# erdc/petsc-dev

Measured on AMD Instinct MI355X. Metric: KSP CG+Jacobi iterations/s x unknowns (3-D 7-pt Poisson, 256^3 rows per GPU); ksp_its_per_sec and spmv_gbps are BASELINE.json's two quantities, higher is better.
Workload: dtype f64

## Files before the change

### petsc-dev_amd/csrc/spmv_csr.hip

```cpp
#include "common.hpp"
#include <map>
#include <array>
#include <memory>
#include <vector>
#include <stdlib.h>
#include <string.h>

#ifndef SPMV_THREADS
#define SPMV_THREADS 256
#endif
#ifndef SPMV_NT
#define SPMV_NT 1
#endif
#ifndef SPMV_REMAP
#define SPMV_REMAP 2
#endif
#ifndef SPMV_CH
#define SPMV_CH 32
#endif
#ifndef SPMV_MINWAVES
#define SPMV_MINWAVES 1
#endif
#ifndef SPMV_SEQ_AVG
#define SPMV_SEQ_AVG 16
#endif
#define SPMV_GJ_CAP 960
#define SPMV_BLOCK_NNZ (8 * SPMV_THREADS)
#define SPMV_BLOCK_CAP (SPMV_BLOCK_NNZ - 2)
#define SPMV_BLOCK_ROWS SPMV_THREADS
#define SPMV_PAIRS (SPMV_BLOCK_NNZ / (2 * SPMV_THREADS))
#define SPMV_WAVES (SPMV_THREADS / MI355X_WAVE)
#if SPMV_NT
#define SPMV_LOAD(p) __builtin_nontemporal_load(p)
#else
#define SPMV_LOAD(p) (*(p))
#endif
static_assert(SPMV_THREADS == 256 && MI355X_WAVE == 64, "one lane per row of a block with byte row markers, 256-entry offset table and 512-entry pattern tables staged one / two per lane");
static_assert(SPMV_REMAP == 0 || SPMV_REMAP == 2, "SPMV_REMAP == 1 (each XCD walks a contiguous eighth of the row blocks) was removed: only the plain kernel ever had it; use 0 or 2");

typedef double v2d __attribute__((ext_vector_type(2)));
typedef int v2i __attribute__((ext_vector_type(2)));

struct mi355x_spmv_plan_s {
  int nrows;
  int nblocks;
  int nlong;
  int2 *d_rowblk;
  int *d_rows;
  unsigned char *d_idx8;
  int *d_offtab;
  int ntab;
  unsigned int *d_prow;
  int *d_pattab;
  int npat, use_pat;
  unsigned int *d_pruns;
  int nruncoded, use_runs;
  int ch;
  unsigned short *d_vrow;
  int *d_vpattab;
  double *d_vpatval;
  int nvpat, vtablen, vpat_valid, use_vpat;
  double *d_dotpart;
  int ndotpart;
  int pairsum;
  int4 *d_rowblk4;
  int *d_goff;
  int *d_gj;
  int ngroups;
  long ngj;
};


static inline int rowblock_grid(int nblocks, int ch) {
  const int per = SPMV_REMAP == 2 ? MI355X_NXCD * ch : 1;
  return ((nblocks + per - 1) / per) * per;
}
__device__ __forceinline__ int rowblock_of_workgroup(int ch) {
  if (SPMV_REMAP != 2) return blockIdx.x;
  const int xcd = blockIdx.x % MI355X_NXCD, slot = blockIdx.x / MI355X_NXCD;
  return ((slot / ch) * MI355X_NXCD + xcd) * ch + (slot % ch);
}

struct row_lanes { int tpr, r, sub; };
__device__ __forceinline__ row_lanes lanes_per_row(int nrows, int nnz, int tid, bool short_rows_one_lane = true) {
  int lg = 0;
  while (lg < 6 && ((nrows * 2) << lg) <= SPMV_THREADS) ++lg;
  if (short_rows_one_lane && nnz <= SPMV_SEQ_AVG * nrows) lg = 0;
  return {1 << lg, tid >> lg, tid & ((1 << lg) - 1)};
}

__device__ __forceinline__ int pair_k(int k0, int tid, int p) { return (k0 & ~1) + 2 * tid + p * 2 * SPMV_THREADS; }
template <typename PAIR, typename T> __device__ __forceinline__ PAIR load_pair(const T *a, int k0, int k1, int k) {
  return SPMV_LOAD(reinterpret_cast<const PAIR *>(a + (k < k1 ? k : (k0 & ~1))));
}
struct pair_src { int kk, s0, s1; };
__device__ __forceinline__ pair_src pair_source(int k, int k0, int k1) {
  const bool in = k < k1;
  const bool v0 = in && k >= k0, v1 = in && (k + 1 < k1);
  return {in ? k : (k0 & ~1), v0 ? 0 : (in ? 1 : (k0 & 1)), v1 ? 1 : (in ? 0 : (k0 & 1))};
}
__device__ __forceinline__ void park_pair(double *stage, int k, int k0, int k1, double a, double b) {
  stage[(k >= k0 && k < k1) ? k - k0 : SPMV_BLOCK_NNZ - 1] = a;
  stage[(k + 1 < k1) ? k + 1 - k0 : SPMV_BLOCK_NNZ - 1] = b;
}

template <class PROD> __device__ __forceinline__ double accumulate8(double sum, int k, int end, int pairsum, PROD prod) {
  if (!pairsum) {
#pragma unroll
    for (int j = 0; j < 8; ++j) { const double u = sum + prod(j); sum = (k + j < end) ? u : sum; }
  } else {
#pragma unroll
    for (int j = 0; j < 8; j += 2) {
      const double pa = prod(j), pb = prod(j + 1);
      const double inc = (k + j + 1 < end) ? pa + pb : pa;
      const double u = sum + inc;
      sum = (k + j < end) ? u : sum;
    }
  }
  return sum;
}
__device__ __forceinline__ double row_sum_lds(const double *prod, int rs, int re, double sum, int pairsum) {
  auto run = [&](int pairs) {
    for (int k = rs; k < re; k += 8) {
      double t[8];
#pragma unroll
      for (int j = 0; j < 8; ++j) t[j] = prod[(k + j < re) ? k + j : re - 1];
      sum = accumulate8(sum, k, re, pairs, [&](int j) { return t[j]; });
    }
  };
  if (!pairsum) run(0); else run(1);
  return sum;
}

template <int ADD> __device__ __forceinline__ double spmv_out(double yv, double t, double dv = 1.0) { return ADD == 3 ? dv * (yv + t) : (ADD == 1 ? yv + t : (ADD == 2 ? yv * t : t)); }
template <int ADD> __device__ __forceinline__ double spmv_empty(double yv, double dv = 1.0) { return ADD == 3 ? dv * yv : (ADD == 1 ? yv : (ADD == 2 ? yv * 0.0 : 0.0)); }
template <int ADD> __device__ __forceinline__ double spmv_fin(double yv, double s, double dv = 1.0) { return ADD == 3 ? dv * s : (ADD == 2 ? yv * s : s); }
static inline int spmv_y_streams(long nrows) { return (size_t)nrows * sizeof(double) >= ((size_t)256 << 20); }
__device__ __forceinline__ void spmv_store(double *p, double v, bool nt) { if (nt) __builtin_nontemporal_store(v, p); else *p = v; }

template <int ADD>
__device__ __forceinline__ double row_result_lds(const double *prod, int tpr, int sub, bool has_row, int rs, int re, double yv, double dv,
                                                 int pairsum, double *dst, bool nt) {
  double res = 0.0;
  if (tpr == 1) {
    if (has_row) { res = spmv_fin<ADD>(yv, row_sum_lds(prod, rs, re, (ADD & 1) ? yv : 0.0, pairsum), dv); spmv_store(dst, res, nt); }
  } else {
    double sum = 0.0;
    if (has_row) for (int k = rs + sub; k < re; k += tpr) sum += prod[k];
    for (int off = tpr >> 1; off > 0; off >>= 1) sum += __shfl_down(sum, off, MI355X_WAVE);
    if (has_row && sub == 0) { res = re == rs ? spmv_empty<ADD>(yv, dv) : spmv_out<ADD>(yv, sum, dv); spmv_store(dst, res, nt); }
  }
  return res;
}

template <int NW> __device__ __forceinline__ double workgroup_sum_ordered(double v) {
  __shared__ double wave_slot[NW];
  const int tid = threadIdx.x;
  v = wave_sum(v);
  if ((tid & (MI355X_WAVE - 1)) == 0) wave_slot[tid / MI355X_WAVE] = v;
  __syncthreads();
  double t = 0.0;
  if (tid == 0) {
    t = wave_slot[0];
// ... 64 lines not shown
    for (int p = 0; p < SPMV_PAIRS; ++p) {
      const pair_src s = pair_source(pair_k(k0, tid, p), k0, k1);
      xa[p] = x[s.s0 ? c[p].y : c[p].x];
      xb[p] = x[s.s1 ? c[p].y : c[p].x];
    }
#pragma unroll
    for (int p = 0; p < SPMV_PAIRS; ++p) park_pair(prod, pair_k(k0, tid, p), k0, k1, v[p].x * xa[p], v[p].y * xb[p]);
  } else {
    for (int k = k0 + tid; k < k1; k += SPMV_THREADS)
      prod[k - k0] = SPMV_LOAD(aa + k) * x[SPMV_LOAD(aj + k)];
  }
  __syncthreads();

  const int rs = r < nrows ? a0 - k0 : 0, re = r < nrows ? a1 - k0 : 0;
  row_result_lds<ADD>(prod, tpr, sub, r < nrows, rs, re, ysum, dv, pairsum, yout + orow, nt);
}

template <int ADD, bool DOT>
__global__ __launch_bounds__(SPMV_THREADS, SPMV_MINWAVES) void spmv_csr_rowblock_idx8_kernel(
    const int2 *__restrict__ rowblk, int nblocks, const int *__restrict__ ai, const unsigned char *__restrict__ idx8,
    const int *__restrict__ offtab_g, int ntab, const double *__restrict__ aa, const double *__restrict__ x,
    const double *yin, double *yout, double *__restrict__ dotpart, int pairsum) {
  __shared__ double prod[SPMV_BLOCK_NNZ];
  __shared__ unsigned char rowof[SPMV_BLOCK_NNZ];
  __shared__ int offtab[256];
  static_assert(!(DOT && ADD != 0), "the x'y by-product is provided for y = A x only");
  const int lb = rowblock_of_workgroup(SPMV_CH);
  if (lb >= nblocks) return;
  const int2 b0 = rowblk[lb];
  const int2 b1 = rowblk[lb + 1];
  const int r0 = b0.x, r1 = b1.x, k0 = b0.y, k1 = b1.y;
  const int nnz = k1 - k0;
  const int nrows = r1 - r0;
  const int tid = threadIdx.x;
  const int tabv = offtab_g[tid];
  (void)ntab;
  if (nnz == 0) {
    if (tid < nrows) yout[r0 + tid] = spmv_empty<ADD>(ADD ? yin[r0 + tid] : 0.0);
    if (DOT && tid == 0) dotpart[lb] = 0.0;
    return;
  }

  const row_lanes rl = lanes_per_row(nrows, nnz, tid);
  const int tpr = rl.tpr, r = rl.r, sub = rl.sub;
  const int rc = r < nrows ? r : nrows - 1;
  const int a0 = ai[r0 + rc], a1 = ai[r0 + rc + 1];
  double ysum = 0.0;
  if (ADD) ysum = yin[r0 + rc];
  double xrow = 0.0;
  if (DOT) xrow = x[r0 + rc];
  v2d v[SPMV_PAIRS];
  unsigned int ix[SPMV_PAIRS];
#pragma unroll
  for (int p = 0; p < SPMV_PAIRS; ++p) {
    v[p] = load_pair<v2d>(aa, k0, k1, pair_k(k0, tid, p));
    ix[p] = load_pair<unsigned short>(idx8, k0, k1, pair_k(k0, tid, p));
  }
  const int rs = r < nrows ? a0 - k0 : 0, re = r < nrows ? a1 - k0 : 0;
  for (int k = rs + sub; k < re; k += tpr) rowof[k] = (unsigned char)r;
  offtab[tid] = tabv;
  __syncthreads();
  double xa[SPMV_PAIRS], xb[SPMV_PAIRS];
#pragma unroll
  for (int p = 0; p < SPMV_PAIRS; ++p) {
    const pair_src s = pair_source(pair_k(k0, tid, p), k0, k1);
    xa[p] = x[r0 + rowof[s.kk + s.s0 - k0] + offtab[(ix[p] >> (8 * s.s0)) & 0xff]];
    xb[p] = x[r0 + rowof[s.kk + s.s1 - k0] + offtab[(ix[p] >> (8 * s.s1)) & 0xff]];
  }
#pragma unroll
  for (int p = 0; p < SPMV_PAIRS; ++p) park_pair(prod, pair_k(k0, tid, p), k0, k1, v[p].x * xa[p], v[p].y * xb[p]);
  __syncthreads();
  const double yval = row_result_lds<ADD>(prod, tpr, sub, r < nrows, rs, re, ysum, 1.0, pairsum, yout + r0 + rc, false);
  if (DOT) {
    const double t = workgroup_sum_ordered<SPMV_WAVES>((r < nrows && sub == 0) ? yval * xrow : 0.0);
    if (tid == 0) dotpart[lb] = t;
  }
}

#define SPMV_PAT_CAP 512
#define SPMV_RUNS 4
#define SPMV_RUN_WORDS (2 * SPMV_RUNS)
#define SPMV_RUN_NONE 0xffffu
static_assert(SPMV_RUNS == 4, "the kernel loads a block's runs as two uint4");
template <int ADD, bool DOT>
__global__ __launch_bounds__(SPMV_THREADS, SPMV_MINWAVES) void spmv_csr_rowblock_pat_kernel(
    const int2 *__restrict__ rowblk, int nblocks, const unsigned int *__restrict__ prow, const uint4 *__restrict__ pruns,
    const int *__restrict__ pattab_g, const double *__restrict__ aa, const double *__restrict__ x, const double *yin, double *yout,
    double *__restrict__ dotpart, int pairsum, int ch, int nty) {
  __shared__ double vs[SPMV_BLOCK_NNZ];
  __shared__ int pattab[SPMV_PAT_CAP];
  const int lb = rowblock_of_workgroup(ch);
  if (lb >= nblocks) return;
  const int2 b0 = rowblk[lb];
  const int2 b1 = rowblk[lb + 1];
  uint4 d0 = make_uint4(0u, SPMV_RUN_NONE, 0u, SPMV_RUN_NONE), d1 = d0;
  if (pruns) { d0 = pruns[2 * (size_t)lb]; d1 = pruns[2 * (size_t)lb + 1]; }
  const int r0 = b0.x, r1 = b1.x, k0 = b0.y, k1 = b1.y;
  const int nrows = r1 - r0;
  const int tid = threadIdx.x;
  const int t0 = pattab_g[tid], t1 = pattab_g[tid + SPMV_THREADS];
  if (k1 == k0) {
    if (tid < nrows) yout[r0 + tid] = spmv_empty<ADD>(ADD ? yin[r0 + tid] : 0.0);
    if (DOT && tid == 0) dotpart[lb] = 0.0;
    return;
  }
  const int rc = tid < nrows ? tid : nrows - 1;
  const bool coded = (d0.y & 0xffffu) == 0u;
  unsigned int pw = d0.x, rn = d0.y;
  if ((unsigned int)rc >= (d0.w & 0xffffu)) { pw = d0.z; rn = d0.w; }
  if ((unsigned int)rc >= (d1.y & 0xffffu)) { pw = d1.x; rn = d1.y; }
  if ((unsigned int)rc >= (d1.w & 0xffffu)) { pw = d1.z; rn = d1.w; }
  if (!coded) pw = prow[r0 + rc];
  const int pst = (int)(pw & 0xffffu);
  const int rs = (int)(pw >> 16) + (rc - (int)(rn & 0xffffu)) * (int)(rn >> 16);
  double ysum = 0.0;
  if (ADD) ysum = yin[r0 + rc];
  v2d v[SPMV_PAIRS];
#pragma unroll
  for (int p = 0; p < SPMV_PAIRS; ++p) v[p] = load_pair<v2d>(aa, k0, k1, pair_k(k0, tid, p));
  pattab[tid] = t0;
  pattab[tid + SPMV_THREADS] = t1;
#pragma unroll
  for (int p = 0; p < SPMV_PAIRS; ++p) park_pair(vs, pair_k(k0, tid, p), k0, k1, v[p].x, v[p].y);
  __syncthreads();
  if (!DOT && tid >= nrows) return;
  const int len = tid < nrows ? (coded ? (int)(rn >> 16) : pattab[pst]) : 0;
  const long xbase = (long)r0 + rc;
  double sum = (ADD == 1) ? ysum : 0.0;
  for (int q0 = 0; q0 < len; q0 += 8) {
    double xv[8], av[8];
#pragma unroll
    for (int j = 0; j < 8; ++j) {
      const int qq = (q0 + j < len) ? q0 + j : len - 1;
      xv[j] = x[xbase + pattab[pst + 1 + qq]];
      av[j] = vs[rs + qq];
    }
    sum = accumulate8(sum, q0, len, pairsum, [&](int j) { return av[j] * xv[j]; });
  }
  const double yv = spmv_fin<ADD>(ysum, sum);
  if (tid < nrows) spmv_store(yout + r0 + tid, yv, nty);
  if (DOT) {
    const double t = workgroup_sum_ordered<SPMV_WAVES>(tid < nrows ? yv * x[xbase] : 0.0);
    if (tid == 0) dotpart[lb] = t;
  }
}

#ifndef SPMV_VPAT_RPL
#define SPMV_VPAT_RPL 4
#endif
#define SPMV_VPAT_ROWS (SPMV_VPAT_RPL * SPMV_THREADS)
#define SPMV_VPAT_MAXROWS (1 << 28)

__device__ __forceinline__ double vpat_row(const int *pattab, const double *patval, int ps, unsigned int rb8, const char *__restrict__ xb,
                                           double sum, int pairsum) {
  const int len = pattab[ps];
  for (int q0 = 0; q0 < len; q0 += 8) {
    double xv[8], av[8];
#pragma unroll
    for (int i = 0; i < 8; ++i) {
      xv[i] = 0.0;
      if (q0 + i < len) xv[i] = *reinterpret_cast<const double *>(xb + (unsigned int)(rb8 + (unsigned int)pattab[ps + 1 + q0 + i]));
      av[i] = patval[ps + 1 + q0 + i];
    }
    sum = accumulate8(sum, q0, len, pairsum, [&](int i) { return av[i] * xv[i]; });
  }
  return sum;
}

template <int ADD, bool DOT>
__global__ __launch_bounds__(SPMV_THREADS) void spmv_csr_valpat_kernel(
    int nrows, const unsigned short *__restrict__ vrow, const int *__restrict__ pattab_g, const double *__restrict__ patval_g, int tablen,
    const double *__restrict__ x, const double *yin, double *yout, double *__restrict__ dotpart, int pairsum) {
  __shared__ int pattab[SPMV_PAT_CAP];
  __shared__ double patval[SPMV_PAT_CAP];
  const int tid = threadIdx.x;
  for (int t = tid; t < tablen; t += SPMV_THREADS) { pattab[t] = pattab_g[t]; patval[t] = patval_g[t]; }
  const long rbase = (long)blockIdx.x * SPMV_VPAT_ROWS + tid;
  int pst[SPMV_VPAT_RPL];
  double yv[SPMV_VPAT_RPL];
#pragma unroll
  for (int j = 0; j < SPMV_VPAT_RPL; ++j) {
    const long row = rbase + (long)j * SPMV_THREADS;
    const long rc = row < nrows ? row : (long)nrows - 1;
    pst[j] = vrow[rc];
    yv[j] = ADD == 2 ? __builtin_nontemporal_load(yin + rc) : (ADD ? yin[rc] : 0.0);
  }
  __syncthreads();
  const char *xb = reinterpret_cast<const char *>(x);
  double res[SPMV_VPAT_RPL];
#pragma unroll
  for (int j = 0; j < SPMV_VPAT_RPL; ++j) {
    const long row = rbase + (long)j * SPMV_THREADS;
    res[j] = 0.0;
    if (row < nrows) res[j] = spmv_fin<ADD>(yv[j], vpat_row(pattab, patval, pst[j], (unsigned int)row * 8u, xb, (ADD == 1) ? yv[j] : 0.0, pairsum));
  }
#pragma unroll
  for (int j = 0; j < SPMV_VPAT_RPL; ++j) {
    const long row = rbase + (long)j * SPMV_THREADS;
    if (row < nrows) yout[row] = res[j];
  }
  if (DOT) {
    double c = 0.0;
#pragma unroll
    for (int j = 0; j < SPMV_VPAT_RPL; ++j) {
      const long row = rbase + (long)j * SPMV_THREADS;
      if (row < nrows) c += res[j] * x[row];
    }
    const double t = workgroup_sum_ordered<SPMV_WAVES>(c);
    if (tid == 0) dotpart[blockIdx.x] = t;
  }
}

template <int ADD>
__global__ __launch_bounds__(SPMV_THREADS, SPMV_MINWAVES) void spmv_csr_rowblock_inode_kernel(
    const int4 *__restrict__ rowblk, int nblocks, const int *__restrict__ ai, const int *__restrict__ goff,
    const int *__restrict__ gj, const double *__restrict__ aa, const double *__restrict__ x, const double *yin, double *yout,
    int pairsum) {
  __shared__ double prod[SPMV_BLOCK_NNZ];
  __shared__ int gjs[SPMV_GJ_CAP + 2];
  __shared__ int rbase[SPMV_BLOCK_ROWS];
  __shared__ unsigned char rowof[SPMV_BLOCK_NNZ];
  static_assert(SPMV_GJ_CAP + 2 <= 4 * SPMV_THREADS, "index staging: two int2 loads per lane");
  const int lb = rowblock_of_workgroup(SPMV_CH);
  if (lb >= nblocks) return;
  const int4 b0 = rowblk[lb];
  const int4 b1 = rowblk[lb + 1];
// ... 260 lines not shown
      }
    }
  }
  __syncthreads();
  return true;
}
template <bool VEC>
__global__ __launch_bounds__(SPMV_THREADS) void csr_zero_columns_kernel(const int2 *__restrict__ rowblk, int nblocks, const int *__restrict__ ai,
                                                                       const int *__restrict__ aj, double *aa, const unsigned *__restrict__ mask,
                                                                       const double *__restrict__ x, double *b) {
  __shared__ double prod[SPMV_BLOCK_NNZ];
  __shared__ unsigned char hit[SPMV_BLOCK_NNZ];
  const int lb = rowblock_of_workgroup(SPMV_CH);
  if (lb >= nblocks) return;
  const int2 b0 = rowblk[lb];
  const int2 b1 = rowblk[lb + 1];
  const int r0 = b0.x, nrows = b1.x - b0.x, k0 = b0.y, k1 = b1.y;
  const int tid = threadIdx.x;
  if (k1 == k0) return;
  if (k1 - k0 > SPMV_BLOCK_CAP) {
    if (zc_listed(mask, r0)) return;
    double bv = 0.0;
    bool touched = false;
    for (int c0 = k0; c0 < k1; c0 += SPMV_BLOCK_NNZ) {
      const int c1 = c0 + SPMV_BLOCK_NNZ < k1 ? c0 + SPMV_BLOCK_NNZ : k1;
      if (!zc_sweep<false>(aj, aa, mask, x, c0, c1, tid, prod, hit, true)) continue;
      if (tid == 0 && b) {
        if (!touched) { bv = b[r0]; touched = true; }
        for (int k = 0; k < c1 - c0; ++k) if (hit[k]) bv = bv - prod[k];
      }
      __syncthreads();
    }
    if (tid == 0 && touched) b[r0] = bv;
    return;
  }
  if (!zc_sweep<VEC>(aj, aa, mask, x, k0, k1, tid, prod, hit, false)) return;
  if (tid < nrows && !zc_listed(mask, r0 + tid)) {
    const int r = r0 + tid;
    const int rs = ai[r] - k0, re = ai[r + 1] - k0;
    double bv = 0.0;
    bool touched = false;
    for (int k = rs; k < re; ++k) {
      if (!hit[k]) continue;
      if (b) {
        if (!touched) { bv = b[r]; touched = true; }
        bv = bv - prod[k];
      }
      aa[k0 + k] = 0.0;
    }
    if (touched) b[r] = bv;
  }
}

enum spmv_form_t { SPMV_PLAIN_SCALAR, SPMV_PLAIN, SPMV_IDX8, SPMV_ROWPAT, SPMV_GROUPED, SPMV_VALPAT };
static spmv_form_t spmv_form(const mi355x_spmv_plan_s *p, const double *aa, const int *aj, bool plain_only = false) {
  const bool a16 = mi355x_aligned16(aa);
  if (!p->d_rows && !plain_only) {
    if (p->vpat_valid && p->use_vpat) return SPMV_VALPAT;
    if (p->d_gj && a16) return SPMV_GROUPED;
    if (p->d_prow && p->use_pat && a16) return SPMV_ROWPAT;
    if (p->d_idx8 && a16) return SPMV_IDX8;
  }
  return (a16 && (((uintptr_t)aj) & 7u) == 0) ? SPMV_PLAIN : SPMV_PLAIN_SCALAR;
}

static inline const uint4 *spmv_runs_of(const mi355x_spmv_plan_s *p) { return p->use_runs ? reinterpret_cast<const uint4 *>(p->d_pruns) : nullptr; }

template <int ADD>
static int launch_spmv(mi355x_handle_t h, mi355x_spmv_plan_t p, const int *ai, const int *aj, const double *aa,
                       const double *x, const double *yin, double *yout, const double *dsc = nullptr) {
  if (p->nblocks == 0) return 0;
  const dim3 grid(rowblock_grid(p->nblocks, SPMV_CH)), block(SPMV_THREADS);
  const spmv_form_t form = spmv_form(p, aa, aj, ADD == 3);
  if constexpr (ADD != 3) switch (form) {
    case SPMV_VALPAT:
      hipLaunchKernelGGL((spmv_csr_valpat_kernel<ADD, false>), dim3((p->nrows + SPMV_VPAT_ROWS - 1) / SPMV_VPAT_ROWS), block, 0, h->stream,
                         p->nrows, p->d_vrow, p->d_vpattab, p->d_vpatval, p->vtablen, x, yin, yout, (double *)nullptr, p->pairsum);
      break;
    case SPMV_GROUPED:
      hipLaunchKernelGGL((spmv_csr_rowblock_inode_kernel<ADD>), grid, block, 0, h->stream, p->d_rowblk4, p->nblocks,
                         ai, p->d_goff, p->d_gj, aa, x, yin, yout, p->pairsum);
      break;
    case SPMV_ROWPAT:
      hipLaunchKernelGGL((spmv_csr_rowblock_pat_kernel<ADD, false>), dim3(rowblock_grid(p->nblocks, p->ch)), block, 0, h->stream, p->d_rowblk,
                         p->nblocks, p->d_prow, spmv_runs_of(p), p->d_pattab, aa, x, yin, yout, (double *)nullptr, p->pairsum, p->ch, spmv_y_streams(p->nrows));
      break;
    case SPMV_IDX8:
      hipLaunchKernelGGL((spmv_csr_rowblock_idx8_kernel<ADD, false>), grid, block, 0, h->stream, p->d_rowblk,
                         p->nblocks, ai, p->d_idx8, p->d_offtab, p->ntab, aa, x, yin, yout, (double *)nullptr, p->pairsum);
      break;
    default: break;
  }
#define SPMV_GO(C, V)                                                                                                  \
  hipLaunchKernelGGL((spmv_csr_rowblock_kernel<ADD, C, V>), grid, block, 0, h->stream, p->d_rowblk, p->nblocks, ai, aj, \
                     aa, x, yin, yout, p->d_rows, p->pairsum, dsc, spmv_y_streams(p->nrows))
  if (form == SPMV_PLAIN)             { if (p->d_rows) SPMV_GO(true, true); else SPMV_GO(false, true); }
  else if (form == SPMV_PLAIN_SCALAR) { if (p->d_rows) SPMV_GO(true, false); else SPMV_GO(false, false); }
#undef SPMV_GO
  MI355X_LAUNCH_CHECK();
  return 0;
}

extern "C" {

static int spmv_plan_create(mi355x_handle_t h, int nrows, const int *ai_host, const int *rows_host, mi355x_spmv_plan_t *plan) {
  std::unique_ptr<mi355x_spmv_plan_s, decltype(&mi355x_spmv_plan_destroy)> p(new mi355x_spmv_plan_s(), mi355x_spmv_plan_destroy);
  p->nrows = nrows;
  p->use_pat = 1; p->use_runs = 1; p->ch = SPMV_CH; p->use_vpat = 1;
  std::vector<int2> rb;
  rb.reserve((size_t)nrows / 128 + 2);
  rb.push_back(make_int2(0, ai_host[0]));
  int r = 0;
  while (r < nrows) {
    const int start = r;
    int nnz = 0;
    while (r < nrows && (r - start) < SPMV_BLOCK_ROWS) {
      const int len = ai_host[r + 1] - ai_host[r];
      if (nnz + len > SPMV_BLOCK_CAP) break;
      nnz += len;
      ++r;
    }
    if (r == start) {
      ++r;
      p->nlong++;
    }
    rb.push_back(make_int2(r, ai_host[r]));
  }
  p->nblocks = (int)rb.size() - 1;
  MI355X_TRY(hipMalloc((void **)&p->d_rowblk, sizeof(int2) * rb.size()));
  MI355X_TRY(hipMemcpyAsync(p->d_rowblk, rb.data(), sizeof(int2) * rb.size(), hipMemcpyHostToDevice, h->stream));
  if (rows_host) {
    MI355X_TRY(hipMalloc((void **)&p->d_rows, sizeof(int) * (size_t)(nrows > 0 ? nrows : 1)));
    MI355X_TRY(hipMemcpyAsync(p->d_rows, rows_host, sizeof(int) * (size_t)nrows, hipMemcpyHostToDevice, h->stream));
  }
  MI355X_TRY(hipStreamSynchronize(h->stream));
  *plan = p.release();
  return 0;
}
int mi355x_spmv_plan_create(mi355x_handle_t h, int nrows, const int *ai_host, const int *rows_host, mi355x_spmv_plan_t *plan) {
  *plan = nullptr;
  return mi355x_guard([&] { return spmv_plan_create(h, nrows, ai_host, rows_host, plan); });
}

static int analysis_threads(int m, int cap) {
  int nth = mi355x_host_threads(cap);
  if (m < 400000) nth = 1;
  const char *e = getenv("MI355X_ANALYSIS_THREADS");
  if (e && atoi(e) > 0) nth = atoi(e) > 64 ? 64 : atoi(e);
  if (nth > m) nth = m > 0 ? m : 1;
  return nth;
}

static void spmv_pattern_runs(int nblocks, const int *rowblk, const unsigned int *prow, const int *pattab, unsigned int *runs, int b_lo, int b_hi, int *ncoded) {
  int coded = 0;
  for (int b = b_lo; b < b_hi; ++b) {
    unsigned int *d = runs + (size_t)SPMV_RUN_WORDS * (size_t)b;
    const int r0 = rowblk[2 * (size_t)b], r1 = rowblk[2 * (size_t)b + 2];
    int n = 0;
    for (int r = r0; r < r1; ++r) {
      if (r > r0 && (prow[r] & 0xffffu) == (prow[r - 1] & 0xffffu)) continue;
      if (n == SPMV_RUNS) { n = SPMV_RUNS + 1; break; }
      d[2 * n] = prow[r];
      d[2 * n + 1] = (unsigned int)(r - r0) | ((unsigned int)pattab[prow[r] & 0xffffu] << 16);
      ++n;
    }
    if (n > SPMV_RUNS) n = 0; else ++coded;
    for (; n < SPMV_RUNS; ++n) { d[2 * n] = 0u; d[2 * n + 1] = SPMV_RUN_NONE; }
// ... 346 lines not shown
}
int mi355x_spmv_plan_group_rows(mi355x_handle_t h, mi355x_spmv_plan_t p, const int *ai_host, const int *aj_host, int nnodes,
                                const int *ns) {
  return mi355x_guard([&] { return spmv_group_rows(h, p, ai_host, aj_host, nnodes, ns); });
}

int mi355x_spmv_plan_set_pairsum(mi355x_spmv_plan_t p, int on) {
  if (p) p->pairsum = on ? 1 : 0;
  return 0;
}

int mi355x_spmv_plan_group_info(mi355x_spmv_plan_t p, int *ngroups, long *nshared_indices, int *pairsum) {
  if (ngroups) *ngroups = p->d_gj ? p->ngroups : 0;
  if (nshared_indices) *nshared_indices = p->d_gj ? p->ngj : 0;
  if (pairsum) *pairsum = p->pairsum;
  return 0;
}

int mi355x_spmv_plan_destroy(mi355x_spmv_plan_t p) {
  if (!p) return 0;
  hipFree(p->d_rowblk);
  hipFree(p->d_idx8);
  hipFree(p->d_offtab);
  hipFree(p->d_prow);
  hipFree(p->d_pattab);
  hipFree(p->d_pruns);
  hipFree(p->d_vrow);
  hipFree(p->d_vpattab);
  hipFree(p->d_vpatval);
  hipFree(p->d_rows);
  hipFree(p->d_dotpart);
  hipFree(p->d_rowblk4);
  hipFree(p->d_goff);
  hipFree(p->d_gj);
  delete p;
  return 0;
}

int mi355x_spmv_plan_is_compressed(mi355x_spmv_plan_t p, int *ntab) {
  if (ntab) *ntab = p->d_idx8 ? p->ntab : 0;
  return 0;
}

int mi355x_spmv_plan_dot_available(mi355x_spmv_plan_t p, const double *aa, int *yes) {
  const spmv_form_t form = spmv_form(p, aa, nullptr);
  if (yes) *yes = (form == SPMV_VALPAT || form == SPMV_ROWPAT || form == SPMV_IDX8) ? 1 : 0;
  return 0;
}

int mi355x_spmv_plan_info(mi355x_spmv_plan_t p, int *nblocks, int *nlong, size_t *workspace_bytes) {
  if (nblocks) *nblocks = p->nblocks;
  if (nlong) *nlong = p->nlong;
  if (workspace_bytes) *workspace_bytes = sizeof(int) * (2 * ((size_t)p->nblocks + 1) + (p->d_rows ? (size_t)p->nrows : 0) +
                                                              (p->d_pruns ? SPMV_RUN_WORDS * (size_t)p->nblocks : 0));
  return 0;
}

int mi355x_spmv_csr(mi355x_handle_t h, mi355x_spmv_plan_t plan, const int *ai, const int *aj, const double *aa,
                    const double *x, double *y) {
  return launch_spmv<0>(h, plan, ai, aj, aa, x, nullptr, y);
}

int mi355x_spmv_csr_scaled(mi355x_handle_t h, mi355x_spmv_plan_t plan, const int *ai, const int *aj, const double *aa,
                           const double *x, const double *d, double *y) {
  return launch_spmv<2>(h, plan, ai, aj, aa, x, d, y);
}

int mi355x_spmv_csr_dot(mi355x_handle_t h, mi355x_spmv_plan_t p, const int *ai, const int *aj, const double *aa,
                        const double *x, double *y) {
  const spmv_form_t form = spmv_form(p, aa, aj);
  if (form != SPMV_VALPAT && form != SPMV_ROWPAT && form != SPMV_IDX8) return (int)hipErrorNotSupported;
  if (p->nblocks == 0) return 0;
  const int nvb = (p->nrows + SPMV_VPAT_ROWS - 1) / SPMV_VPAT_ROWS;
  { const size_t need = (size_t)(p->nblocks > nvb ? p->nblocks : nvb);
    if (!p->d_dotpart) MI355X_TRY(hipMalloc((void **)&p->d_dotpart, sizeof(double) * need)); }
  const dim3 block(SPMV_THREADS);
  const double *const no_yin = nullptr;
  switch (form) {
    case SPMV_VALPAT:
      hipLaunchKernelGGL((spmv_csr_valpat_kernel<0, true>), dim3(nvb), block, 0, h->stream, p->nrows, p->d_vrow, p->d_vpattab,
                         p->d_vpatval, p->vtablen, x, no_yin, y, p->d_dotpart, p->pairsum);
      break;
    case SPMV_ROWPAT:
      hipLaunchKernelGGL((spmv_csr_rowblock_pat_kernel<0, true>), dim3(rowblock_grid(p->nblocks, p->ch)), block, 0, h->stream, p->d_rowblk,
                         p->nblocks, p->d_prow, spmv_runs_of(p), p->d_pattab, aa, x, no_yin, y, p->d_dotpart, p->pairsum, p->ch, spmv_y_streams(p->nrows));
      break;
    default:
      hipLaunchKernelGGL((spmv_csr_rowblock_idx8_kernel<0, true>), dim3(rowblock_grid(p->nblocks, SPMV_CH)), block, 0, h->stream, p->d_rowblk,
                         p->nblocks, ai, p->d_idx8, p->d_offtab, p->ntab, aa, x, no_yin, y, p->d_dotpart, p->pairsum);
      break;
  }
  p->ndotpart = form == SPMV_VALPAT ? nvb : p->nblocks;
  MI355X_LAUNCH_CHECK();
  return 0;
}
int mi355x_spmv_dot_finish(mi355x_handle_t h, mi355x_spmv_plan_t p, double *out) {
  if (p->nblocks == 0 || !p->d_dotpart || p->ndotpart <= 0) { MI355X_TRY(hipMemsetAsync(out, 0, sizeof(double), h->stream)); return 0; }
  hipLaunchKernelGGL(dot_partials_kernel, dim3(1), dim3(1024), 0, h->stream, p->d_dotpart, p->ndotpart, out);
  MI355X_LAUNCH_CHECK();
  return 0;
}

int mi355x_spmv_csr_add(mi355x_handle_t h, mi355x_spmv_plan_t plan, const int *ai, const int *aj, const double *aa,
                        const double *x, const double *y, double *z) {
  return launch_spmv<1>(h, plan, ai, aj, aa, x, y, z);
}

int mi355x_spmv_csr_add_scaled(mi355x_handle_t h, mi355x_spmv_plan_t plan, const int *ai, const int *aj, const double *aa,
                               const double *x, const double *y, const double *d, double *z) {
  if (!d || !y) return (int)hipErrorInvalidValue;
  return launch_spmv<3>(h, plan, ai, aj, aa, x, y, z, d);
}

static int spmv_bsr_planned_impl(mi355x_handle_t h, mi355x_spmv_plan_t p, int bs, const int *ai, const int *aj,
                                 const double *aa, const double *x, const double *yin, double *y, bool xlds) {
  if (p->nblocks == 0) return 0;
  const dim3 grid(rowblock_grid(p->nblocks, SPMV_CH)), block(SPMV_THREADS);
#define BSR_GO(B) do { if (xlds) hipLaunchKernelGGL((bsr_rowblock_kernel<B, true>), grid, block, 0, h->stream, p->d_rowblk, p->nblocks, ai, aj, aa, x, yin, y); \
                       else hipLaunchKernelGGL((bsr_rowblock_kernel<B, false>), grid, block, 0, h->stream, p->d_rowblk, p->nblocks, ai, aj, aa, x, yin, y); } while (0)
  switch (bs) {
    case 2: BSR_GO(2); break;
    case 3: BSR_GO(3); break;
    case 4: BSR_GO(4); break;
    case 5: BSR_GO(5); break;
    case 6: BSR_GO(6); break;
    case 7: BSR_GO(7); break;
    case 8: BSR_GO(8); break;
    default: return (int)hipErrorInvalidValue;
  }
#undef BSR_GO
  MI355X_LAUNCH_CHECK();
  return 0;
}
int mi355x_spmv_bsr_planned_form(mi355x_handle_t h, mi355x_spmv_plan_t p, int bs, int x_in_lds, const int *ai, const int *aj,
                                 const double *aa, const double *x, double *y) {
  return spmv_bsr_planned_impl(h, p, bs, ai, aj, aa, x, nullptr, y, x_in_lds != 0);
}
int mi355x_spmv_bsr_planned(mi355x_handle_t h, mi355x_spmv_plan_t p, int bs, const int *ai, const int *aj,
                            const double *aa, const double *x, double *y) {
  return spmv_bsr_planned_impl(h, p, bs, ai, aj, aa, x, nullptr, y, MI355X_BSR_XLDS_DEFAULT != 0);
}
int mi355x_spmv_bsr_planned_add(mi355x_handle_t h, mi355x_spmv_plan_t p, int bs, const int *ai, const int *aj,
                                const double *aa, const double *x, const double *y, double *z) {
  return spmv_bsr_planned_impl(h, p, bs, ai, aj, aa, x, y, z, MI355X_BSR_XLDS_DEFAULT != 0);
}

int mi355x_csr_assemble(mi355x_handle_t h, int nseg, const int *segptr, const int *segslot, const int *order, const double *v, double *aa) {
  if (nseg <= 0) return 0;
  hipLaunchKernelGGL(csr_assemble_kernel, dim3((nseg + MI355X_BLOCK - 1) / MI355X_BLOCK), dim3(MI355X_BLOCK), 0, h->stream, nseg, segptr, segslot, order, v, aa);
  MI355X_LAUNCH_CHECK();
  return 0;
}

int mi355x_csr_diagonal_scale(mi355x_handle_t h, int m, const int *ai, const int *aj, double *aa, const double *l, const double *r) {
  if (m <= 0 || (!l && !r)) return 0;
  hipLaunchKernelGGL(csr_diagscale_kernel, dim3((m + MI355X_BLOCK - 1) / MI355X_BLOCK), dim3(MI355X_BLOCK), 0, h->stream, m, ai, aj, aa, l, r);
  MI355X_LAUNCH_CHECK();
  return 0;
}

int mi355x_csr_get_diagonal(mi355x_handle_t h, int m, const int *ai, const int *aj, const double *aa, double *d) {
  if (m <= 0) return 0;
  hipLaunchKernelGGL(csr_diag_kernel, dim3((m + MI355X_BLOCK - 1) / MI355X_BLOCK), dim3(MI355X_BLOCK), 0, h->stream, m,
                     ai, aj, aa, d);
  MI355X_LAUNCH_CHECK();
  return 0;
}
// ... 70 lines not shown
```

Measured before the change: 39620.

## Pipeline multiple row blocks per workgroup in pattern SpMV kernel

New measurement: 39520. About the same (-0.2%).

```diff
diff --git a/petsc-dev_amd/csrc/spmv_csr.hip b/petsc-dev_amd/csrc/spmv_csr.hip
--- a/petsc-dev_amd/csrc/spmv_csr.hip
+++ b/petsc-dev_amd/csrc/spmv_csr.hip
@@ -4,6 +4,7 @@
 #include <memory>
 #include <vector>
 #include <stdlib.h>
+#include <limits.h>
 #include <string.h>
 
 #ifndef SPMV_THREADS
@@ -71,14 +72,16 @@
 };
 
 
-static inline int rowblock_grid(int nblocks, int ch) {
-  const int per = SPMV_REMAP == 2 ? MI355X_NXCD * ch : 1;
-  return ((nblocks + per - 1) / per) * per;
-}
-__device__ __forceinline__ int rowblock_of_workgroup(int ch) {
-  if (SPMV_REMAP != 2) return blockIdx.x;
+static inline int rowblock_grid(int nblocks, int ch, int nb = 1) {
+  if (SPMV_REMAP != 2) return (nblocks + nb - 1) / nb;
+  const int per = MI355X_NXCD * ch;
+  return ((nblocks + per - 1) / per) * MI355X_NXCD * ((ch + nb - 1) / nb);
+}
+__device__ __forceinline__ int rowblock_of_workgroup(int ch, int nb = 1, int j = 0) {
+  if (SPMV_REMAP != 2) return blockIdx.x * nb + j;
   const int xcd = blockIdx.x % MI355X_NXCD, slot = blockIdx.x / MI355X_NXCD;
-  return ((slot / ch) * MI355X_NXCD + xcd) * ch + (slot % ch);
+  const int wpr = (ch + nb - 1) / nb, pos = (slot % wpr) * nb + j;
+  return pos < ch ? ((slot / wpr) * MI355X_NXCD + xcd) * ch + pos : INT_MAX;
 }
 
 struct row_lanes { int tpr, r, sub; };
@@ -309,66 +312,98 @@
 #define SPMV_RUN_WORDS (2 * SPMV_RUNS)
 #define SPMV_RUN_NONE 0xffffu
 static_assert(SPMV_RUNS == 4, "the kernel loads a block's runs as two uint4");
+#ifndef SPMV_PAT_NB
+#define SPMV_PAT_NB 1
+#endif
+#define SPMV_PAT_MINWAVES 8
+struct pat_head { int lb, r0, nrows, k0, k1; unsigned int pw[SPMV_RUNS], rn[SPMV_RUNS]; };
+__device__ __forceinline__ pat_head pat_block_head(int j, int nblocks, int ch, const int2 *__restrict__ rowblk, const uint4 *__restrict__ pruns) {
+  pat_head h = {INT_MAX, 0, 0, 0, 0, {0u, 0u, 0u, 0u}, {SPMV_RUN_NONE, SPMV_RUN_NONE, SPMV_RUN_NONE, SPMV_RUN_NONE}};
+  if (j >= SPMV_PAT_NB) return h;
+  const int lb = rowblock_of_workgroup(ch, SPMV_PAT_NB, j);
+  if (lb >= nblocks) return h;
+  const int2 b0 = rowblk[lb];
+  const int2 b1 = rowblk[lb + 1];
+  if (pruns) {
+    const uint4 d0 = pruns[2 * (size_t)lb], d1 = pruns[2 * (size_t)lb + 1];
+    h.pw[0] = d0.x; h.rn[0] = d0.y; h.pw[1] = d0.z; h.rn[1] = d0.w;
+    h.pw[2] = d1.x; h.rn[2] = d1.y; h.pw[3] = d1.z; h.rn[3] = d1.w;
+  }
+  h.lb = lb; h.r0 = b0.x; h.nrows = b1.x - b0.x; h.k0 = b0.y; h.k1 = b1.y;
+  return h;
+}
+__device__ __forceinline__ void pat_load_values(v2d (&v)[SPMV_PAIRS], const double *__restrict__ aa, const pat_head &h, int tid) {
+  if (h.k1 == h.k0) return;
+#pragma unroll
+  for (int p = 0; p < SPMV_PAIRS; ++p) v[p] = load_pair<v2d>(aa, h.k0, h.k1, pair_k(h.k0, tid, p));
+}
 template <int ADD, bool DOT>
-__global__ __launch_bounds__(SPMV_THREADS, SPMV_MINWAVES) void spmv_csr_rowblock_pat_kernel(
+__global__ __launch_bounds__(SPMV_THREADS, SPMV_PAT_MINWAVES) void spmv_csr_rowblock_pat_kernel(
     const int2 *__restrict__ rowblk, int nblocks, const unsigned int *__restrict__ prow, const uint4 *__restrict__ pruns,
     const int *__restrict__ pattab_g, const double *__restrict__ aa, const double *__restrict__ x, const double *yin, double *yout,
     double *__restrict__ dotpart, int pairsum, int ch, int nty) {
   __shared__ double vs[SPMV_BLOCK_NNZ];
   __shared__ int pattab[SPMV_PAT_CAP];
-  const int lb = rowblock_of_workgroup(ch);
-  if (lb >= nblocks) return;
-  const int2 b0 = rowblk[lb];
-  const int2 b1 = rowblk[lb + 1];
-  uint4 d0 = make_uint4(0u, SPMV_RUN_NONE, 0u, SPMV_RUN_NONE), d1 = d0;
-  if (pruns) { d0 = pruns[2 * (size_t)lb]; d1 = pruns[2 * (size_t)lb + 1]; }
-  const int r0 = b0.x, r1 = b1.x, k0 = b0.y, k1 = b1.y;
-  const int nrows = r1 - r0;
   const int tid = threadIdx.x;
+  pat_head cur = pat_block_head(0, nblocks, ch, rowblk, pruns), nxt = pat_block_head(1, nblocks, ch, rowblk, pruns);
+  if (cur.lb >= nblocks) return;
   const int t0 = pattab_g[tid], t1 = pattab_g[tid + SPMV_THREADS];
-  if (k1 == k0) {
-    if (tid < nrows) yout[r0 + tid] = spmv_empty<ADD>(ADD ? yin[r0 + tid] : 0.0);
-    if (DOT && tid == 0) dotpart[lb] = 0.0;
-    return;
-  }
-  const int rc = tid < nrows ? tid : nrows - 1;
-  const bool coded = (d0.y & 0xffffu) == 0u;
-  unsigned int pw = d0.x, rn = d0.y;
-  if ((unsigned int)rc >= (d0.w & 0xffffu)) { pw = d0.z; rn = d0.w; }
-  if ((unsigned int)rc >= (d1.y & 0xffffu)) { pw = d1.x; rn = d1.y; }
-  if ((unsigned int)rc >= (d1.w & 0xffffu)) { pw = d1.z; rn = d1.w; }
-  if (!coded) pw = prow[r0 + rc];
-  const int pst = (int)(pw & 0xffffu);
-  const int rs = (int)(pw >> 16) + (rc - (int)(rn & 0xffffu)) * (int)(rn >> 16);
-  double ysum = 0.0;
-  if (ADD) ysum = yin[r0 + rc];
   v2d v[SPMV_PAIRS];
-#pragma unroll
-  for (int p = 0; p < SPMV_PAIRS; ++p) v[p] = load_pair<v2d>(aa, k0, k1, pair_k(k0, tid, p));
+  pat_load_values(v, aa, cur, tid);
   pattab[tid] = t0;
   pattab[tid + SPMV_THREADS] = t1;
-#pragma unroll
-  for (int p = 0; p < SPMV_PAIRS; ++p) park_pair(vs, pair_k(k0, tid, p), k0, k1, v[p].x, v[p].y);
-  __syncthreads();
-  if (!DOT && tid >= nrows) return;
-  const int len = tid < nrows ? (coded ? (int)(rn >> 16) : pattab[pst]) : 0;
-  const long xbase = (long)r0 + rc;
-  double sum = (ADD == 1) ? ysum : 0.0;
-  for (int q0 = 0; q0 < len; q0 += 8) {
-    double xv[8], av[8];
-#pragma unroll
-    for (int j = 0; j < 8; ++j) {
-      const int qq = (q0 + j < len) ? q0 + j : len - 1;
-      xv[j] = x[xbase + pattab[pst + 1 + qq]];
-      av[j] = vs[rs + qq];
-    }
-    sum = accumulate8(sum, q0, len, pairsum, [&](int j) { return av[j] * xv[j]; });
-  }
-  const double yv = spmv_fin<ADD>(ysum, sum);
-  if (tid < nrows) spmv_store(yout + r0 + tid, yv, nty);
-  if (DOT) {
-    const double t = workgroup_sum_ordered<SPMV_WAVES>(tid < nrows ? yv * x[xbase] : 0.0);
-    if (tid == 0) dotpart[lb] = t;
+  bool staged = false;
+#pragma unroll
+  for (int j = 0; j < SPMV_PAT_NB; ++j) {
+    const int lb = cur.lb, r0 = cur.r0, nrows = cur.nrows, k0 = cur.k0, k1 = cur.k1;
+    if (lb >= nblocks) break;
+    const bool work = k1 != k0;
+    const int rc = tid < nrows ? tid : nrows - 1;
+    const bool coded = (cur.rn[0] & 0xffffu) == 0u;
+    unsigned int pw = cur.pw[0], rn = cur.rn[0];
+#pragma unroll
+    for (int u = 1; u < SPMV_RUNS; ++u) if ((unsigned int)rc >= (cur.rn[u] & 0xffffu)) { pw = cur.pw[u]; rn = cur.rn[u]; }
+    double ysum = 0.0;
+    int pst = 0, rs = 0;
+    if (work) {
+      if (!coded) pw = prow[r0 + rc];
+      if (ADD) ysum = yin[r0 + rc];
+      pst = (int)(pw & 0xffffu);
+      rs = (int)(pw >> 16) + (rc - (int)(rn & 0xffffu)) * (int)(rn >> 16);
+      if (!DOT && staged) __syncthreads();
+#pragma unroll
+      for (int p = 0; p < SPMV_PAIRS; ++p) park_pair(vs, pair_k(k0, tid, p), k0, k1, v[p].x, v[p].y);
+      __syncthreads();
+      staged = true;
+    }
+    pat_load_values(v, aa, nxt, tid);
+    const pat_head nn = pat_block_head(j + 2, nblocks, ch, rowblk, pruns);
+    if (!work) {
+      if (tid < nrows) yout[r0 + tid] = spmv_empty<ADD>(ADD ? yin[r0 + tid] : 0.0);
+      if (DOT && tid == 0) dotpart[lb] = 0.0;
+    } else if (DOT || tid < nrows) {
+      const int len = tid < nrows ? (coded ? (int)(rn >> 16) : pattab[pst]) : 0;
+      const long xbase = (long)r0 + rc;
+      double sum = (ADD == 1) ? ysum : 0.0;
+      for (int q0 = 0; q0 < len; q0 += 8) {
+        double xv[8], av[8];
+#pragma unroll
+        for (int i = 0; i < 8; ++i) {
+          const int qq = (q0 + i < len) ? q0 + i : len - 1;
+          xv[i] = x[xbase + pattab[pst + 1 + qq]];
+          av[i] = vs[rs + qq];
+        }
+        sum = accumulate8(sum, q0, len, pairsum, [&](int i) { return av[i] * xv[i]; });
+      }
+      const double yv = spmv_fin<ADD>(ysum, sum);
+      if (tid < nrows) spmv_store(yout + r0 + tid, yv, nty);
+      if (DOT) {
+        const double t = workgroup_sum_ordered<SPMV_WAVES>(tid < nrows ? yv * x[xbase] : 0.0);
+        if (tid == 0) dotpart[lb] = t;
+      }
+    }
+    cur = nxt;
+    nxt = nn;
   }
 }
 
@@ -795,7 +830,7 @@
                          ai, p->d_goff, p->d_gj, aa, x, yin, yout, p->pairsum);
       break;
     case SPMV_ROWPAT:
-      hipLaunchKernelGGL((spmv_csr_rowblock_pat_kernel<ADD, false>), dim3(rowblock_grid(p->nblocks, p->ch)), block, 0, h->stream, p->d_rowblk,
+      hipLaunchKernelGGL((spmv_csr_rowblock_pat_kernel<ADD, false>), dim3(rowblock_grid(p->nblocks, p->ch, SPMV_PAT_NB)), block, 0, h->stream, p->d_rowblk,
                          p->nblocks, p->d_prow, spmv_runs_of(p), p->d_pattab, aa, x, yin, yout, (double *)nullptr, p->pairsum, p->ch, spmv_y_streams(p->nrows));
       break;
     case SPMV_IDX8:
@@ -1308,7 +1343,7 @@
                          p->d_vpatval, p->vtablen, x, no_yin, y, p->d_dotpart, p->pairsum);
       break;
     case SPMV_ROWPAT:
-      hipLaunchKernelGGL((spmv_csr_rowblock_pat_kernel<0, true>), dim3(rowblock_grid(p->nblocks, p->ch)), block, 0, h->stream, p->d_rowblk,
+      hipLaunchKernelGGL((spmv_csr_rowblock_pat_kernel<0, true>), dim3(rowblock_grid(p->nblocks, p->ch, SPMV_PAT_NB)), block, 0, h->stream, p->d_rowblk,
                          p->nblocks, p->d_prow, spmv_runs_of(p), p->d_pattab, aa, x, no_yin, y, p->d_dotpart, p->pairsum, p->ch, spmv_y_streams(p->nrows));
       break;
     default:
```
